# musyoku/wavenet

Measured on AMD Instinct MI355X. Metric: audio samples/sec: train fwd+bwd, 4x10-layer dilated stack (cfg2), higher is better.
Workload: dtype f32 storage+accumulate / fp16x2 split products (2^-21)

## Files before the change

wavenet_amd/csrc/mfma_gemm_b3.hip:

```cpp
#include "mfma_gemm.hpp"
#include "split_w.hpp"
#include "h2_ops.hpp"
#include <type_traits>

namespace wn {

template <bool WMAX>
__global__ void k_split_w(CGArgs a, int mode, int mtiles, int chunks_per_src, __bf16* __restrict__ img, int one) {
    if (WMAX) {
        const float mw = split_w_tile<true>(a, mode, mtiles, chunks_per_src, img, one, (int)blockIdx.x, 1.f);
        if (threadIdx.x == 0) atomicMax(const_cast<unsigned*>(a.wmax_dev), __float_as_uint(mw));
    } else {
        split_w_tile<false>(a, mode, mtiles, chunks_per_src, img, one, (int)blockIdx.x, one == 3 ? h2_scale(a.wmax_dev, kH2ScaleW) : 1.f);
    }
}

__device__ __forceinline__ int b3_ch(int r, int h) { return (r & 3) + 8 * (r >> 2) + 4 * h; }

struct RowMap { long long row[4]; bool ok[4]; };

__device__ __forceinline__ RowMap row_map(long long no, bool nvalid, int lane) {
    RowMap m;
#pragma unroll
    for (int it = 0; it < 4; ++it) {
// ... 600 lines not shown
    const long long img_stride = (long long)mtiles * kH2qTB;
    auto dma_half = [&](int s) {
        const int ss = s < nhalf ? s : nhalf - 1;
        const char* base = reinterpret_cast<const char*>(img) + (long long)(ss >> 1) * img_stride + (ss & 1) * kH2qHalf;
#pragma unroll
        for (int tt = 0; tt < 2; ++tt)
            asm_dma2(tile_off[tt], base, lds0 + ((s & 3) * MT + swave + 4 * tt) * kH2qHalf);
    };
    f32x4 xr[4][2];
    const int rs0 = rbase + a.soff[0];
    const bool rv0 = rs0 >= 0 && rs0 < a.rows_src_per_b;
    const float msk0 = rv0 ? 1.f : 0.f;
    const unsigned x_off = (unsigned)(((rb0 + (rv0 ? rs0 : 0)) * (a.ldx ? a.ldx : a.K[0]) + 8 * h) * 4);
    const char* x0 = reinterpret_cast<const char*>(a.X[0]);
    auto load_x = [&](int s, auto slot_tag) {
        constexpr int slot = decltype(slot_tag)::value;
        const int ss = s < nhalf ? s : nhalf - 1;
        const char* base = x0 + (long long)(ss >> 1) * x_stride + (ss & 1) * 64;
        asm_load16s(xr[slot][0], x_off, base);
        asm_load16s(xr[slot][1], x_off + 16, base);
    };
    f16x8 xh[2], xm[2];
    auto split_one = [&](const f32x4 (&raw)[2], float ms, int e, f16x8& oh, f16x8& om) {
        const float v = raw[e >> 2][e & 3];
        _Float16 a0, a1;
        split2h(act_apply_t<ACT>(v) * (ms * h2sx), a0, a1);
        oh[e] = a0; om[e] = a1;
    };
    using I0 = std::integral_constant<int, 0>;
    using I1 = std::integral_constant<int, 1>;
    using I2 = std::integral_constant<int, 2>;
    using I3 = std::integral_constant<int, 3>;
    load_x(0, I0{});
    asm volatile("s_waitcnt vmcnt(0)" : "+v"(xr[0][0]), "+v"(xr[0][1]) : : "memory");
#pragma unroll
    for (int e = 0; e < 8; ++e) split_one(xr[0], msk0, e, xh[0], xm[0]);
    asm volatile("" : "+v"(xh[0]), "+v"(xm[0]));
    dma_half(0); load_x(1, I1{});
    dma_half(1); load_x(2, I2{});
    dma_half(2); load_x(3, I3{});

    auto step = [&](int s, auto p_tag) {
        constexpr int p = decltype(p_tag)::value;
        constexpr int set = p & 1, nxt = 1 - set;
        constexpr int rn = (p + 1) & 3;
        asm volatile("s_waitcnt vmcnt(12)" : "+v"(xr[rn][0]), "+v"(xr[rn][1]) : : "memory");
        const float ms = msk0;
        asm volatile("s_waitcnt lgkmcnt(0)" ::: "memory");
        __builtin_amdgcn_s_barrier();
        dma_half(s + 3);
        const char* Ab = ldsq + (p * MT) * kH2qHalf + lane * 16;
        f16x8 fr[2][2];
        auto ldA = [&](int mt, f16x8 (&f)[2]) {
            f[0] = *reinterpret_cast<const f16x8*>(Ab + mt * kH2qHalf);
            f[1] = *reinterpret_cast<const f16x8*>(Ab + mt * kH2qHalf + 1024);
        };
        ldA(0, fr[0]);
#pragma unroll
        for (int mt = 0; mt < MT; ++mt) {
            f16x8 (&f)[2] = fr[mt & 1];
            asm volatile("" ::"v"(f[0]));
            asm volatile("" ::"v"(f[1]));
            if (mt + 1 < MT) ldA(mt + 1, fr[(mt + 1) & 1]);
            __builtin_amdgcn_sched_barrier(0);
            split_one(xr[rn], ms, mt, nxt ? xh[1] : xh[0], nxt ? xm[1] : xm[0]);
            acc[mt] = __builtin_amdgcn_mfma_f32_32x32x16_f16(f[1], xh[set], acc[mt], 0, 0, 0);
            acc[mt] = __builtin_amdgcn_mfma_f32_32x32x16_f16(f[0], xm[set], acc[mt], 0, 0, 0);
            acc[mt] = __builtin_amdgcn_mfma_f32_32x32x16_f16(f[0], xh[set], acc[mt], 0, 0, 0);
            __builtin_amdgcn_sched_barrier(0);
        }
        asm volatile("" : "+v"(xh[nxt]), "+v"(xm[nxt]));
        load_x(s + 4, p_tag);
    };
    for (int s = 0; s < nhalf; s += 4) {
        step(s, I0{});
        step(s + 1, I1{});
        step(s + 2, I2{});
        step(s + 3, I3{});
    }
    asm volatile("s_waitcnt vmcnt(0)"
                 : "+v"(xr[0][0]), "+v"(xr[0][1]), "+v"(xr[1][0]), "+v"(xr[1][1]), "+v"(xr[2][0]), "+v"(xr[2][1]),
                   "+v"(xr[3][0]), "+v"(xr[3][1])
                 :
                 : "memory");
#pragma unroll
    for (int mt = 0; mt < MT; ++mt)
#pragma unroll
        for (int r = 0; r < 16; ++r) acc[mt][r] *= 1.f / (h2sw * h2sx);
    __syncthreads();
    float* patch = reinterpret_cast<float*>(ldsq) + wave * 1024;
    const RowMap rm = row_map(no, nvalid, lane);
#pragma unroll
    for (int mt = 0; mt < MT; ++mt) {
        if (t0 + mt >= mtiles) break;
        float* __restrict__ og = (MODE == 2) ? a.out[t0 + mt] : a.out[0];
        const int col = (MODE == 2) ? 0 : (t0 + mt) * 32;
        float4 t[4], v[4], u[4];
#pragma unroll
        for (int q = 0; q < 4; ++q) t[q] = make_float4(acc[mt][4 * q], acc[mt][4 * q + 1], acc[mt][4 * q + 2], acc[mt][4 * q + 3]);
        if (MODE == 0 && a.gate_x) {
            rows_load(a.gate_x, a.ldo, col, rm, lane, v);
            rows_to_tile(patch, lane, v, u);
#pragma unroll
            for (int q = 0; q < 4; ++q) {
                t[q].x *= act_grad(u[q].x, a.gate_act); t[q].y *= act_grad(u[q].y, a.gate_act);
                t[q].z *= act_grad(u[q].z, a.gate_act); t[q].w *= act_grad(u[q].w, a.gate_act);
            }
        }
        if (MODE == 0 && a.residual) {
            rows_load(a.residual, a.ldo, col, rm, lane, v);
            rows_to_tile(patch, lane, v, u);
#pragma unroll
            for (int q = 0; q < 4; ++q) { t[q].x += u[q].x; t[q].y += u[q].y; t[q].z += u[q].z; t[q].w += u[q].w; }
        }
        if (a.accumulate) {
            rows_load(og, a.ldo, col, rm, lane, v);
            rows_to_tile(patch, lane, v, u);
#pragma unroll
            for (int q = 0; q < 4; ++q) { t[q].x += u[q].x; t[q].y += u[q].y; t[q].z += u[q].z; t[q].w += u[q].w; }
        }
        tile_store_rows(patch, lane, t, og, a.ldo, col, rm);
    }
}

static constexpr int kWsTile = 32 * 1024;
static constexpr int kWsLds = 2 * kWsTile + 8 * 4096;
static constexpr int kWsAhead = 2;

__global__ __launch_bounds__(512, 1) void k_dz_ws(CGArgs a, const __bf16* __restrict__ img, int mtiles, int ntiles, int nranges) {
    extern __shared__ __attribute__((aligned(16))) char ldsw[];
    const float h2sx = h2_scale(a.xmax_dev, kH2ScaleX);
    const float h2sw = h2_scale(a.wmax_dev, kH2ScaleW);
    const int tid = threadIdx.x, lane = tid & 63;
    const int wave = __builtin_amdgcn_readfirstlane(tid >> 6);
    const int j = lane & 31, h = lane >> 5;
    int range, grp;
    {
        const int ng = (mtiles + 7) >> 3;
        const int id = blockIdx.x;
        const int full = nranges & ~7;
        if (id < full * ng) {
            const int g = id / (8 * ng), rem = id - g * 8 * ng;
            range = g * 8 + (rem & 7);
            grp = rem >> 3;
        } else {
            const int t = id - full * ng;
            grp = t % ng;
            range = full + t / ng;
        }
    }
    const int t_lo = (int)((long long)range * ntiles / nranges), t_hi = (int)((long long)(range + 1) * ntiles / nranges);
    if (t_lo >= t_hi) return;
    const int layer = grp * 8 + wave;
    const bool live = layer < mtiles;
    const int N = (int)a.N, rows_out = a.rows_out_per_b, rows_src = a.rows_src_per_b, shift = a.off + a.soff[0];
    const int ldo = a.ldo;
    const long long ldx = a.ldx ? a.ldx : a.K[0];
    const float* __restrict__ X = a.X[0];
    float* __restrict__ og = a.out[live ? layer : 0];

    f16x8 A[16][2];
    {
        const char* ip = reinterpret_cast<const char*>(img) + (long long)(live ? layer : mtiles - 1) * kH2qTB + lane * 16;
#pragma unroll
        for (int kk = 0; kk < 16; ++kk)
#pragma unroll
            for (int pl = 0; pl < 2; ++pl)
                A[kk][pl] = *reinterpret_cast<const f16x8*>(ip + (long long)(kk >> 1) * mtiles * kH2qTB + (kk & 1) * kH2qHalf + pl * 1024);
    }

    auto advance = [&](int& n, int& b, int& r, int by) {
        n += by; r += by;
        const bool wrap = r >= rows_out;
        r -= wrap ? rows_out : 0;
        b += wrap ? 1 : 0;
    };
    const int lcol = (tid & 7) | ((tid >> 7) << 3), kseg = (tid >> 3) & 15;
    int ln = t_lo * 32 + lcol, lb = ln / rows_out, lr = ln - lb * rows_out;
    float4 raw[4];
    float rsc = 0.f;
    auto load_raw = [&]() {
        const int rs = lr + shift;
        const bool rv = ln < N && rs >= 0 && rs < rows_src;
        rsc = rv ? h2sx : 0.f;
        const float* p = X + (rv ? (long long)lb * rows_src + rs : 0ll) * ldx + 16 * kseg;
#pragma unroll
        for (int i = 0; i < 4; ++i) raw[i] = reinterpret_cast<const float4*>(p)[i];
        advance(ln, lb, lr, 32);
    };
    auto split_write = [&](char* buf) {
        float v[16];
#pragma unroll
        for (int e = 0; e < 16; ++e) {
            const float x = (e & 3) == 0 ? raw[e >> 2].x : (e & 3) == 1 ? raw[e >> 2].y : (e & 3) == 2 ? raw[e >> 2].z : raw[e >> 2].w;
            v[e] = fminf(fmaxf(x * rsc, -65000.f), 65000.f);
        }
        H2Op o;
        lb_split16(v, 1.f, o);
        char* d = buf + kseg * 2048 + lcol * 16;
        *reinterpret_cast<f16x8*>(d) = o.h[0];
        *reinterpret_cast<f16x8*>(d + 512) = o.h[1];
        *reinterpret_cast<f16x8*>(d + 1024) = o.m[0];
        *reinterpret_cast<f16x8*>(d + 1536) = o.m[1];
    };
    float* patch = reinterpret_cast<float*>(ldsw + 2 * kWsTile) + wave * 1024;
    const int orows = a.out_rows_per_b ? a.out_rows_per_b : rows_out, orow0 = a.out_rows_per_b ? a.out_row0 : 0;
    int sn[4], sb[4], sr[4];
#pragma unroll
    for (int it = 0; it < 4; ++it) {
        sn[it] = t_lo * 32 + it * 8 + (lane >> 3);
        sb[it] = sn[it] / rows_out;
        sr[it] = sn[it] - sb[it] * rows_out;
    }
    float4 pv0, pv1, pv2, pv3;
    auto patch_read = [&]() {
        pv0 = *reinterpret_cast<const float4*>(patch_rows(patch, lane, 0));
        pv1 = *reinterpret_cast<const float4*>(patch_rows(patch, lane, 1));
        pv2 = *reinterpret_cast<const float4*>(patch_rows(patch, lane, 2));
        pv3 = *reinterpret_cast<const float4*>(patch_rows(patch, lane, 3));
    };
    auto store_rows = [&](const float4 v, int& n, int& b, int& r, bool en) {
        const long long no = (long long)b * orows + orow0 + r;
        if (en && n < N) *reinterpret_cast<float4*>(og + no * ldo + ((lane & 7) << 2)) = v;
        advance(n, b, r, en ? 32 : 0);
    };
    auto store_tile = [&](bool en) {
        store_rows(pv0, sn[0], sb[0], sr[0], en);
        store_rows(pv1, sn[1], sb[1], sr[1], en);
        store_rows(pv2, sn[2], sb[2], sr[2], en);
        store_rows(pv3, sn[3], sb[3], sr[3], en);
    };

    f32x16 acc;
#pragma unroll
    for (int r = 0; r < 16; ++r) acc[r] = 0.f;
    const float inv = 1.f / (h2sw * h2sx);

    auto step = [&](auto live_tag, int t) {
        constexpr bool LIVE = decltype(live_tag)::value;
        char* nxt = ldsw + ((t - t_lo + 1) & 1) * kWsTile;
        const char* rd = ldsw + ((t - t_lo) & 1) * kWsTile + lane * 16;
        f16x8 fr[kWsAhead + 1][2];
        auto ldB = [&](int kk, f16x8 (&f)[2]) {
            f[0] = *reinterpret_cast<const f16x8*>(rd + kk * 2048);
            f[1] = *reinterpret_cast<const f16x8*>(rd + kk * 2048 + 1024);
        };
        if (LIVE) {
#pragma unroll
            for (int kk = 0; kk < kWsAhead; ++kk) ldB(kk, fr[kk]);
        }
#pragma unroll
        for (int kk = 0; kk < 16; ++kk) {
            if (LIVE) {
                f16x8 (&f)[2] = fr[kk % (kWsAhead + 1)];
                asm volatile("" ::"v"(f[0]));
                asm volatile("" ::"v"(f[1]));
                if (kk + kWsAhead < 16) ldB(kk + kWsAhead, fr[(kk + kWsAhead) % (kWsAhead + 1)]);
                __builtin_amdgcn_sched_barrier(0);
                acc = __builtin_amdgcn_mfma_f32_32x32x16_f16(A[kk][1], f[0], acc, 0, 0, 0);
                acc = __builtin_amdgcn_mfma_f32_32x32x16_f16(A[kk][0], f[1], acc, 0, 0, 0);
                acc = __builtin_amdgcn_mfma_f32_32x32x16_f16(A[kk][0], f[0], acc, 0, 0, 0);
                __builtin_amdgcn_sched_barrier(0);
            }
            if (kk == 5) {
                split_write(nxt);
                __builtin_amdgcn_sched_barrier(0);
            }
            if (kk == 6 && LIVE) {
                patch_read();
                __builtin_amdgcn_sched_barrier(0);
            }
            if (kk == 7) {
                if (LIVE) store_tile(t > t_lo);
                load_raw();
                __builtin_amdgcn_sched_barrier(0);
            }
        }
        if (LIVE) {
#pragma unroll
            for (int q = 0; q < 4; ++q)
                *reinterpret_cast<float4*>(patch_tile(patch, j, h, q)) =
                    make_float4(acc[4 * q] * inv, acc[4 * q + 1] * inv, acc[4 * q + 2] * inv, acc[4 * q + 3] * inv);
#pragma unroll
            for (int r = 0; r < 16; ++r) acc[r] = 0.f;
        }
        asm volatile("s_waitcnt lgkmcnt(0)" ::: "memory");
        __builtin_amdgcn_s_barrier();
    };

    load_raw();
    split_write(ldsw);
    load_raw();
    asm volatile("s_waitcnt lgkmcnt(0)" ::: "memory");
    __builtin_amdgcn_s_barrier();
    if (live) {
        for (int t = t_lo; t < t_hi; ++t) step(std::true_type{}, t);
        patch_read();
        store_tile(true);
    } else {
        for (int t = t_lo; t < t_hi; ++t) step(std::false_type{}, t);
    }
}

int launch_colgemm_b3(Call& c, CGArgs& a, int mode, int nprob, hipStream_t s) {
    if (mode != 0 && mode != 2 && mode != 3 && mode != 4 && mode != 5 && mode != 6) return WN_ESHAPE;
    if (mode == 6 && !(c.fp16x2() && a.M == 256 && a.nsrc == 1 && a.xent_target && a.xent_loss && a.out[0] &&
                       cdiv(a.N, 128) <= kXentBlocks))
        return WN_ESHAPE;
    int mtiles, nchunks, cps;
    if (mode == 0 || mode >= 3) {
        if (a.M % 32) return WN_ESHAPE;
        if ((mode == 3 || mode == 5) && a.nsrc > WN_GATE_TAPS) return WN_ESHAPE;
        if (mode == 5 && !(c.one_term() && a.M == 128 && a.ldo == 128)) return WN_ESHAPE;
        for (int i = 0; i < a.nsrc; ++i)
            if (a.K[i] != a.K[0] || a.K[i] % 32) return WN_ESHAPE;
        mtiles = ((mode == 3 || mode == 5) ? 2 : 1) * a.M / 32;
        cps = a.K[0] / 32;
        nchunks = a.nsrc * cps;
    } else {
        if (a.M != 32 || a.K[0] % 32) return WN_ESHAPE;
        mtiles = nprob;
        cps = a.K[0] / 32;
        nchunks = cps;
    }
    const bool one = c.one_term();
    const bool h2 = c.fp16x2() && ((a.h2_ok || a.xmax_dev) && (mode == 0 || mode == 2) || mode == 6);
    const size_t bytes = (size_t)nchunks * mtiles * (one ? kTileBytes / 3 : (h2 ? kTileBytes * 2 / 3 : kTileBytes));
    const size_t bytes2 = mode == 5 ? (size_t)16 * (kTileBytes / 3) : 0;
    const __bf16* pimg = nullptr; const unsigned* pwmax = nullptr;
    const bool planned = plan_split_image(c, a, mode, mtiles, cps, nchunks, one ? 1 : (h2 ? 3 : 0), bytes, &pimg, &pwmax);
    __bf16* img = planned ? const_cast<__bf16*>(pimg)
                          : reinterpret_cast<__bf16*>(c.scratch(bytes + bytes2, "the split weight image"));
    if (!img) return WN_EARG;
    if (planned) {
        a.wmax_dev = pwmax;
    } else {
    if (h2) {
        bool fresh = false;
        unsigned* wm = c.word(reinterpret_cast<const char*>(a.W[0]) + (((unsigned)mode & 7u) << 8 | ((unsigned)a.nsrc & 255u)), &fresh, s);
        if (!wm) return WN_EARG;
        a.wmax_dev = wm;
        if (fresh) hipLaunchKernelGGL(k_split_w<true>, dim3(nchunks * mtiles), dim3(256), 0, s, a, mode, mtiles, cps, img, 3);
    }
    hipLaunchKernelGGL(k_split_w<false>, dim3(nchunks * mtiles), dim3(256), 0, s, a, mode, mtiles, cps, img, one ? 1 : (h2 ? 3 : 0));
    }
    if (mode == 5) {
        if (!a.proj_W || !a.residual || !a.gate_z || a.act != WN_ACT_NONE || mtiles != 8) {
            wn::set_error("colgemm_b3: fused-layer mode needs Wp, the residual input, z and 128 gate channels");
            return WN_EARG;
        }
        CGArgs b{};
        b.nsrc = 1; b.W[0] = a.proj_W; b.wsm[0] = 128; b.wsk = 1; b.K[0] = 128; b.M = 128;
        __bf16* img2 = reinterpret_cast<__bf16*>(reinterpret_cast<char*>(img) + bytes);
        hipLaunchKernelGGL(k_split_w<false>, dim3(16), dim3(256), 0, s, b, 0, 4, 4, img2, 1);
        hipLaunchKernelGGL((k_colgemm_b3<5, WN_ACT_NONE, 1, 8>), dim3(cdiv(a.N, 128)), dim3(256), 0, s, a,
                           (const __bf16*)img, mtiles, nchunks, cps, (const __bf16*)img2);
        WN_LAUNCH_CHECK();
        return WN_OK;
    }
    if (h2 && mode == 2 && nchunks == 8 && a.ldo == 32 && !a.accumulate && !c.flag(WN_EXEC_NO_PIPELINED_GEMM) &&
        a.N < (1ll << 30) && a.rows_out_per_b >= 32 &&
        (a.N / a.rows_out_per_b + 2) * (long long)(a.out_rows_per_b > a.rows_out_per_b ? a.out_rows_per_b : a.rows_out_per_b) < (1ll << 31)) {
        int dev = 0;
        WN_HIP(hipGetDevice(&dev));
        static int capacity[64];
        if (dev < 0 || dev >= 64) { wn::set_error("colgemm_b3: device index %d", dev); return WN_ESHAPE; }
        if (!capacity[dev]) {
            int n_cu = 0, per_cu = 0;
            WN_HIP(hipDeviceGetAttribute(&n_cu, hipDeviceAttributeMultiprocessorCount, dev));
            WN_HIP(hipFuncSetAttribute(reinterpret_cast<const void*>(k_dz_ws), hipFuncAttributeMaxDynamicSharedMemorySize, kWsLds));
            WN_HIP(hipOccupancyMaxActiveBlocksPerMultiprocessor(&per_cu, k_dz_ws, 512, kWsLds));
            capacity[dev] = n_cu * per_cu > 0 ? n_cu * per_cu : -1;
        }
        const int ng = cdiv(mtiles, 8), ntiles = cdiv(a.N, 32);
        int nranges = capacity[dev] / ng;
        if (nranges > ntiles) nranges = ntiles;
        if (nranges >= 1) {
            hipLaunchKernelGGL(k_dz_ws, dim3(ng * nranges), dim3(512), kWsLds, s, a, (const __bf16*)img, mtiles, ntiles, nranges);
            WN_LAUNCH_CHECK();
            return WN_OK;
        }
    }
    const bool mt8 = (one || h2) && mtiles >= 8;
    dim3 grid(cdiv(a.N, 128) * cdiv(mtiles, mt8 ? 8 : 4));
    if (mode == 6) {
#define X_LAUNCH(ACT_, ROWS_) hipLaunchKernelGGL((k_colgemm_b3<6, ACT_, 3, 8, ROWS_>), grid, dim3(256), 0, s, a, (const __bf16*)img, \
                                                 mtiles, nchunks, cps, (const __bf16*)nullptr)
        if (c.flag(WN_EXEC_HEAD_ROW_NLL)) {
            if (a.act == WN_ACT_RELU) X_LAUNCH(WN_ACT_RELU, true);
            else if (a.act == WN_ACT_ELU) X_LAUNCH(WN_ACT_ELU, true);
            else X_LAUNCH(WN_ACT_NONE, true);
        } else if (a.act == WN_ACT_RELU) X_LAUNCH(WN_ACT_RELU, false);
        else if (a.act == WN_ACT_ELU) X_LAUNCH(WN_ACT_ELU, false);
        else X_LAUNCH(WN_ACT_NONE, false);
#undef X_LAUNCH
        WN_LAUNCH_CHECK();
        return WN_OK;
    }
#define CG_LAUNCH(MODE_, ACT_)                                                                                          \
    do {                                                                                                                \
        if (mt8) hipLaunchKernelGGL((k_colgemm_b3<MODE_, ACT_, 1, 8>), grid, dim3(256), 0, s, a, (const __bf16*)img,    \
                                    mtiles, nchunks, cps, (const __bf16*)nullptr);                                      \
        else if (one) hipLaunchKernelGGL((k_colgemm_b3<MODE_, ACT_, 1, 4>), grid, dim3(256), 0, s, a,                   \
                                         (const __bf16*)img, mtiles, nchunks, cps, (const __bf16*)nullptr);             \
        else hipLaunchKernelGGL((k_colgemm_b3<MODE_, ACT_, 6, 4>), grid, dim3(256), 0, s, a, (const __bf16*)img,        \
                                mtiles, nchunks, cps, (const __bf16*)nullptr);                                          \
    } while (0)
#define CG_LAUNCH_H2(MODE_, ACT_)                                                                                       \
    do {                                                                                                                \
        if (mt8) hipLaunchKernelGGL((k_colgemm_b3<MODE_, ACT_, 3, 8>), grid, dim3(256), 0, s, a, (const __bf16*)img,    \
                                    mtiles, nchunks, cps, (const __bf16*)nullptr);                                      \
        else hipLaunchKernelGGL((k_colgemm_b3<MODE_, ACT_, 3, 4>), grid, dim3(256), 0, s, a, (const __bf16*)img,        \
                                mtiles, nchunks, cps, (const __bf16*)nullptr);                                          \
    } while (0)
    long long x_stride = 128;
    bool lean = h2 && mt8 && mode == 0 && (nchunks & 1) == 0 && !c.flag(WN_EXEC_NO_PIPELINED_GEMM) &&
                (a.N / a.rows_out_per_b + 1) * (long long)a.rows_src_per_b * (a.ldx ? a.ldx : a.K[0]) * 4 < (1ll << 32);
    if (lean && mode == 0 && a.nsrc > 1) {
        x_stride = (const char*)a.X[1] - (const char*)a.X[0];
        lean = cps == 1;
        for (int i = 1; i < a.nsrc && lean; ++i)
            lean = a.soff[i] == a.soff[0] && a.K[i] == a.K[0] && (const char*)a.X[i] - (const char*)a.X[i - 1] == x_stride;
    } else if (lean && mode == 0) {
        lean = a.nsrc == 1;
    }
    if (lean) {
        WN_MAX_LDS_ONCE(kH2qLds, k_colgemm_h2q<0, WN_ACT_NONE>, k_colgemm_h2q<0, WN_ACT_RELU>, k_colgemm_h2q<0, WN_ACT_ELU>);
#define Q_LAUNCH(MODE_, ACT_)                                                                                 \
    hipLaunchKernelGGL((k_colgemm_h2q<MODE_, ACT_>), grid, dim3(256), kH2qLds, s, a, (const __bf16*)img, mtiles, nchunks, x_stride)
        if (a.act == WN_ACT_RELU) Q_LAUNCH(0, WN_ACT_RELU);
        else if (a.act == WN_ACT_ELU) Q_LAUNCH(0, WN_ACT_ELU);
        else Q_LAUNCH(0, WN_ACT_NONE);
#undef Q_LAUNCH
        WN_LAUNCH_CHECK();
        return WN_OK;
    }
    if (h2) {
        if (mode == 2) CG_LAUNCH_H2(2, WN_ACT_NONE);
        else if (a.act == WN_ACT_RELU) CG_LAUNCH_H2(0, WN_ACT_RELU);
        else if (a.act == WN_ACT_ELU) CG_LAUNCH_H2(0, WN_ACT_ELU);
        else CG_LAUNCH_H2(0, WN_ACT_NONE);
        WN_LAUNCH_CHECK();
        return WN_OK;
    }
#undef CG_LAUNCH_H2
    if (mode == 3) {
        if (a.act != WN_ACT_NONE || !a.gate_z) { wn::set_error("colgemm_b3: gate mode takes no activation and needs gate_z"); return WN_EARG; }
        CG_LAUNCH(3, WN_ACT_NONE);
    } else if (mode == 4) {
        if (a.act != WN_ACT_NONE || !a.gate_z || !a.gate_f || !a.gate_s) { wn::set_error("colgemm_b3: gate-backward mode needs f, s and the output"); return WN_EARG; }
        CG_LAUNCH(4, WN_ACT_NONE);
    } else if (mode == 0) {
        if (a.outmax_dev) plan_xmax_written(c, a.out[0]);
        if (a.act == WN_ACT_RELU) CG_LAUNCH(0, WN_ACT_RELU);
        else if (a.act == WN_ACT_ELU) CG_LAUNCH(0, WN_ACT_ELU);
        else if (a.act == WN_ACT_NONE) CG_LAUNCH(0, WN_ACT_NONE);
        else { wn::set_error("colgemm_b3: unknown activation %d", a.act); return WN_EARG; }
    } else {
        if (a.act != WN_ACT_NONE) { wn::set_error("colgemm_b3: multi-problem mode takes no activation"); return WN_EARG; }
        CG_LAUNCH(2, WN_ACT_NONE);
    }
#undef CG_LAUNCH
    WN_LAUNCH_CHECK();
    return WN_OK;
}

template <int MT, bool HAS_B2, int ACT, bool ONE>
__global__ __launch_bounds__(256, 2) void k_wgrad_b3(WGArgs a) {
    __shared__ __attribute__((aligned(16))) char lds[MT * kTileBytes];
    constexpr int NF = MT / 2 > 0 ? MT / 2 : 1;
    const int tid = threadIdx.x, lane = tid & 63, wv = tid >> 6;
    const int j = lane & 31, h = lane >> 5;
    const int p = blockIdx.y * 4 + wv;
    const bool active = p < a.nprob;
    const int m0 = blockIdx.z * (MT * 32);
    const int b = blockIdx.x / a.wgs_per_b;
    const int r_begin = (blockIdx.x - b * a.wgs_per_b) * a.rows_per_wg;
    const int r_end = min(a.rows_A_per_b, r_begin + a.rows_per_wg);
    const float* __restrict__ Ab = a.A + ((long long)b * a.rows_A_per_b) * a.lda + m0;
    const float* __restrict__ Bb = a.Bp[active ? p : 0] + ((long long)b * a.rows_B_per_b + a.off) * a.ldb + j;
    const float* __restrict__ B2b = a.B2p[active ? p : 0] ? a.B2p[active ? p : 0] + ((long long)b * a.rows_B_per_b + a.off) * a.ldb + j : nullptr;
    f32x16 acc[MT];
#pragma unroll
    for (int mt = 0; mt < MT; ++mt)
#pragma unroll
        for (int r = 0; r < 16; ++r) acc[mt][r] = 0.f;

    float ar[NF][8], br[2][8], b2r[2][8];
    const float* __restrict__ B2s = HAS_B2 ? B2b : Bb;
    const float amask = active ? 1.f : 0.f;
    int fm[NF], fg[NF];
#pragma unroll
    for (int it = 0; it < NF; ++it) {
        const int f = it * 256 + tid;
        fm[it] = f % (MT * 32);
        fg[it] = f / (MT * 32);
    }
    auto issue = [&](int r0) {
        const bool full = r0 + 32 <= r_end && r0 + a.off >= 0 && r0 + 31 + a.off < a.rows_B_per_b;
        if (full) {
#pragma unroll
            for (int it = 0; it < NF; ++it) {
                const float* ap = Ab + (long long)(r0 + 8 * (fg[it] & 3)) * a.lda + fm[it];
#pragma unroll
                for (int jj = 0; jj < 8; ++jj) ar[it][jj] = ap[(long long)jj * a.lda];
            }
            const float* bp = Bb + (long long)(r0 + 8 * h) * a.ldb;
            const float* b2p = B2s + (long long)(r0 + 8 * h) * a.ldb;
#pragma unroll
            for (int ks = 0; ks < 2; ++ks)
#pragma unroll
                for (int jj = 0; jj < 8; ++jj) {
                    br[ks][jj] = bp[(long long)(16 * ks + jj) * a.ldb];
                    if (HAS_B2) b2r[ks][jj] = b2p[(long long)(16 * ks + jj) * a.ldb];
                }
            return;
        }
#pragma unroll
        for (int it = 0; it < NF; ++it)
#pragma unroll
            for (int jj = 0; jj < 8; ++jj) {
                const int r = r0 + 8 * (fg[it] & 3) + jj;
                const int rc = r < r_end ? r : r_end - 1;
                ar[it][jj] = Ab[(long long)rc * a.lda + fm[it]];
            }
#pragma unroll
        for (int ks = 0; ks < 2; ++ks)
#pragma unroll
            for (int jj = 0; jj < 8; ++jj) {
                const int r = r0 + 16 * ks + 8 * h + jj;
                int rc = r < r_end ? r : r_end - 1;
                if (rc + a.off < 0) rc = -a.off;
                if (rc + a.off >= a.rows_B_per_b) rc = a.rows_B_per_b - 1 - a.off;
                br[ks][jj] = Bb[(long long)rc * a.ldb];
                if (HAS_B2) b2r[ks][jj] = B2s[(long long)rc * a.ldb];
            }
    };
    if (r_begin < r_end) issue(r_begin);
    for (int r0 = r_begin; r0 < r_end; r0 += 32) {
        bf16x8 ah[NF], am[NF], al[NF], bh[2], bm[2], bl[2];
        const bool edge = !(r0 + 32 <= r_end && r0 + a.off >= 0 && r0 + 31 + a.off < a.rows_B_per_b);
#pragma unroll
        for (int it = 0; it < NF; ++it)
#pragma unroll
            for (int e = 0; e < 8; ++e) {
                float av = ar[it][e];
                if (edge) av *= (r0 + 8 * (fg[it] & 3) + e) < r_end ? 1.f : 0.f;
                __bf16 x0, x1, x2;
                split3(av, x0, x1, x2);
                ah[it][e] = x0; am[it][e] = x1; al[it][e] = x2;
            }
#pragma unroll
        for (int ks = 0; ks < 2; ++ks)
#pragma unroll
            for (int e = 0; e < 8; ++e) {
                float bv = act_apply_t<ACT>(br[ks][e]) * amask;
                if (HAS_B2) bv *= b2r[ks][e];
                if (edge) {
                    const int rb = r0 + 16 * ks + 8 * h + e;
                    bv *= (rb < r_end && rb + a.off >= 0 && rb + a.off < a.rows_B_per_b) ? 1.f : 0.f;
                }
                __bf16 x0, x1, x2;
                split3(bv, x0, x1, x2);
                bh[ks][e] = x0; bm[ks][e] = x1; bl[ks][e] = x2;
            }
        __syncthreads();
#pragma unroll
        for (int it = 0; it < NF; ++it) {
            const int f = it * 256 + tid;
            const int m = f % (MT * 32), g = f / (MT * 32);
            if (MT >= 2 || g < 4) {
                char* d = lds + (m >> 5) * kTileBytes + ((g >> 1) * 3) * 1024 + ((m & 31) + 32 * (g & 1)) * 16;
                *reinterpret_cast<bf16x8*>(d) = ah[it];
                *reinterpret_cast<bf16x8*>(d + 1024) = am[it];
                *reinterpret_cast<bf16x8*>(d + 2048) = al[it];
            }
        }
        __syncthreads();
        if (r0 + 32 < r_end) issue(r0 + 32);
        const char* Al = lds + lane * 16;
#pragma unroll
        for (int mt = 0; mt < MT; ++mt) {
#pragma unroll
            for (int ks = 0; ks < 2; ++ks) {
                const char* q = Al + mt * kTileBytes + ks * 3 * 1024;
                const bf16x8 xh = *reinterpret_cast<const bf16x8*>(q);
                const bf16x8 xm = *reinterpret_cast<const bf16x8*>(q + 1024);
                const bf16x8 xl = *reinterpret_cast<const bf16x8*>(q + 2048);
                if (!ONE) {
                    acc[mt] = __builtin_amdgcn_mfma_f32_32x32x16_bf16(xl, bh[ks], acc[mt], 0, 0, 0);
                    acc[mt] = __builtin_amdgcn_mfma_f32_32x32x16_bf16(xh, bl[ks], acc[mt], 0, 0, 0);
                    acc[mt] = __builtin_amdgcn_mfma_f32_32x32x16_bf16(xm, bm[ks], acc[mt], 0, 0, 0);
                    acc[mt] = __builtin_amdgcn_mfma_f32_32x32x16_bf16(xm, bh[ks], acc[mt], 0, 0, 0);
                    acc[mt] = __builtin_amdgcn_mfma_f32_32x32x16_bf16(xh, bm[ks], acc[mt], 0, 0, 0);
                }
                acc[mt] = __builtin_amdgcn_mfma_f32_32x32x16_bf16(xh, bh[ks], acc[mt], 0, 0, 0);
            }
        }
    }
    if (!active) return;
    if (a.fixed_part) {
        const long long M = (long long)gridDim.z * (MT * 32);
        float* __restrict__ q = a.fixed_part + (((long long)blockIdx.x * a.nprob + p) * M) * 32 + j;
#pragma unroll
        for (int mt = 0; mt < MT; ++mt)
#pragma unroll
            for (int r = 0; r < 16; ++r) q[(long long)(m0 + mt * 32 + b3_ch(r, h)) * 32] = acc[mt][r];
        return;
    }
    float* __restrict__ o = a.out[p];
#pragma unroll
    for (int mt = 0; mt < MT; ++mt)
#pragma unroll
        for (int r = 0; r < 16; ++r)
            atomicAdd(o + (long long)(m0 + mt * 32 + b3_ch(r, h)) * a.ldo + (long long)j * (a.osk ? a.osk : 1), acc[mt][r]);
}

template <bool HAS_B2, int ACT, int TM>
__global__ __launch_bounds__(512, 1) void k_wgrad_b3w(WGArgs a) {
    constexpr int MT = 8;
    constexpr bool ONE = TM == 1;
    constexpr bool H2 = TM == 3;
    const float h2sa = H2 ? h2_scale(a.amax_dev, 1.f) : 1.f;
    const float h2sb = H2 ? h2_scale(a.bmax_dev, kH2ScaleX) : 1.f;
    extern __shared__ __attribute__((aligned(16))) char ldsw[];
    const int tid = threadIdx.x, lane = tid & 63, wv = tid >> 6;
    const int j = lane & 31, h = lane >> 5;
    const int p = blockIdx.y * 8 + wv;
    const bool active = p < a.nprob;
    const int off = a.off + a.offp[active ? p : 0];
    const int b = blockIdx.x / a.wgs_per_b;
    const int r_begin = (blockIdx.x - b * a.wgs_per_b) * a.rows_per_wg;
    const int r_end = min(a.rows_A_per_b, r_begin + a.rows_per_wg);
    const float* __restrict__ Ab = a.A + ((long long)b * a.rows_A_per_b) * a.lda;
    const float* __restrict__ Bb = a.Bp[active ? p : 0] + ((long long)b * a.rows_B_per_b + off) * a.ldb + j;
    const float* __restrict__ B2b = a.B2p[active ? p : 0] ? a.B2p[active ? p : 0] + ((long long)b * a.rows_B_per_b + off) * a.ldb + j : nullptr;
    f32x16 acc[MT];
#pragma unroll
    for (int mt = 0; mt < MT; ++mt)
#pragma unroll
        for (int r = 0; r < 16; ++r) acc[mt][r] = 0.f;

    const int fm = tid & 255;
    const int fhh = tid >> 8;
    float ar[2][8], br[2][8], b2r[2][8];
    const float* __restrict__ B2s = HAS_B2 ? B2b : Bb;
    auto issue = [&](int r0) {
        const bool full = r0 + 32 <= r_end && r0 + off >= 0 && r0 + 31 + off < a.rows_B_per_b;
        if (full) {
#pragma unroll
            for (int ks = 0; ks < 2; ++ks) {
                const float* ap = Ab + (long long)(r0 + 16 * ks + 8 * fhh) * a.lda + fm;
#pragma unroll
                for (int jj = 0; jj < 8; ++jj) ar[ks][jj] = ap[(long long)jj * a.lda];
            }
            const float* bp = Bb + (long long)(r0 + 8 * h) * a.ldb;
            const float* b2p = B2s + (long long)(r0 + 8 * h) * a.ldb;
#pragma unroll
            for (int ks = 0; ks < 2; ++ks)
#pragma unroll
                for (int jj = 0; jj < 8; ++jj) {
                    br[ks][jj] = bp[(long long)(16 * ks + jj) * a.ldb];
                    if (HAS_B2) b2r[ks][jj] = b2p[(long long)(16 * ks + jj) * a.ldb];
                }
            return;
        }
#pragma unroll
        for (int ks = 0; ks < 2; ++ks)
#pragma unroll
            for (int jj = 0; jj < 8; ++jj) {
                const int r = r0 + 16 * ks + 8 * fhh + jj;
                const int rc = r < r_end ? r : r_end - 1;
                ar[ks][jj] = Ab[(long long)rc * a.lda + fm];
            }
#pragma unroll
        for (int ks = 0; ks < 2; ++ks)
#pragma unroll
            for (int jj = 0; jj < 8; ++jj) {
                const int r = r0 + 16 * ks + 8 * h + jj;
                int rc = r < r_end ? r : r_end - 1;
                if (rc + off < 0) rc = -off;
// ... 388 lines not shown
```

Measured before the change: 48.37 million.

## Add persistent weight-stationary pipelined kernel for 256x256 three-term dX GEMM

Result: faster. 48.88 million, median of 6 (+1.0%).

```diff
diff --git a/wavenet_amd/csrc/mfma_gemm_b3.hip b/wavenet_amd/csrc/mfma_gemm_b3.hip
--- a/wavenet_amd/csrc/mfma_gemm_b3.hip
+++ b/wavenet_amd/csrc/mfma_gemm_b3.hip
@@ -926,6 +926,186 @@
     }
 }
 
+static constexpr int kDxTile = 48 * 1024;
+static constexpr int kDxLds = 2 * kDxTile + 4 * 4096;
+static constexpr int kDxAhead = 2;
+
+template <int ACT>
+__global__ __launch_bounds__(256, 1) void k_dx_ws(CGArgs a, const __bf16* __restrict__ img, int ntiles, int nranges) {
+    extern __shared__ __attribute__((aligned(16))) char ldsx[];
+    const int tid = threadIdx.x, lane = tid & 63;
+    const int wave = __builtin_amdgcn_readfirstlane(tid >> 6);
+    const int j = lane & 31, h = lane >> 5;
+    int range, grp;
+    {
+        const int id = blockIdx.x;
+        const int full = nranges & ~7;
+        if (id < full * 2) {
+            const int g = id >> 4, rem = id & 15;
+            range = g * 8 + (rem & 7);
+            grp = rem >> 3;
+        } else {
+            const int t = id - full * 2;
+            grp = t & 1;
+            range = full + (t >> 1);
+        }
+    }
+    const int t_lo = (int)((long long)range * ntiles / nranges), t_hi = (int)((long long)(range + 1) * ntiles / nranges);
+    if (t_lo >= t_hi) return;
+    const int mtile = grp * 4 + wave;
+    const int N = (int)a.N;
+    const float* __restrict__ X = a.X[0];
+    const float* __restrict__ G = a.gate_x;
+    float* __restrict__ og = a.out[0] + mtile * 32 + ((lane & 7) << 2);
+    unsigned* const outmax = a.outmax_dev;
+
+    bf16x8 A[16][3];
+    {
+        const char* ip = reinterpret_cast<const char*>(img) + (long long)mtile * kTileBytes + lane * 16;
+#pragma unroll
+        for (int kk = 0; kk < 16; ++kk)
+#pragma unroll
+            for (int pl = 0; pl < 3; ++pl)
+                A[kk][pl] = *reinterpret_cast<const bf16x8*>(ip + (long long)(kk >> 1) * 8 * kTileBytes + (kk & 1) * (kTileBytes / 2) + pl * 1024);
+    }
+
+    const int lcol = (tid & 7) | ((tid >> 7) << 3), kseg = (tid >> 3) & 15;
+    int ln = t_lo * 32 + lcol;
+    float4 raw[2][4];
+    bool rok[2] = {false, false};
+    auto load_raw = [&]() {
+#pragma unroll
+        for (int c2 = 0; c2 < 2; ++c2) {
+            const int n = ln + 16 * c2;
+            rok[c2] = n < N;
+            const float* p = X + (long long)(rok[c2] ? n : 0) * 256 + 16 * kseg;
+#pragma unroll
+            for (int i = 0; i < 4; ++i) raw[c2][i] = reinterpret_cast<const float4*>(p)[i];
+        }
+        ln += 32;
+    };
+    auto split_write = [&](char* buf, int q) {
+        const int c2 = q >> 1, half = q & 1;
+        bf16x8 ph, pm, pl;
+#pragma unroll
+        for (int e = 0; e < 8; ++e) {
+            const float4 r = raw[c2][2 * half + (e >> 2)];
+            const float x = (e & 3) == 0 ? r.x : (e & 3) == 1 ? r.y : (e & 3) == 2 ? r.z : r.w;
+            __bf16 hh, mm, ll;
+            split3(rok[c2] ? x : 0.f, hh, mm, ll);
+            ph[e] = hh; pm[e] = mm; pl[e] = ll;
+        }
+        char* d = buf + kseg * 3072 + (lcol + 16 * c2 + 32 * half) * 16;
+        *reinterpret_cast<bf16x8*>(d) = ph;
+        *reinterpret_cast<bf16x8*>(d + 1024) = pm;
+        *reinterpret_cast<bf16x8*>(d + 2048) = pl;
+    };
+    float* patch = reinterpret_cast<float*>(ldsx + 2 * kDxTile) + wave * 1024;
+    float4 pv[4], gv[4];
+    float omax = 0.f;
+    auto patch_read = [&]() {
+#pragma unroll
+        for (int it = 0; it < 4; ++it) pv[it] = *reinterpret_cast<const float4*>(patch_rows(patch, lane, it));
+    };
+    auto load_gate = [&](int t) {
+        if (ACT == WN_ACT_NONE) return;
+#pragma unroll
+        for (int it = 0; it < 4; ++it) {
+            const int n = t * 32 + it * 8 + (lane >> 3);
+            gv[it] = *reinterpret_cast<const float4*>(G + (long long)(n < N ? n : 0) * 256 + mtile * 32 + ((lane & 7) << 2));
+        }
+    };
+    auto store_tile = [&](int t) {
+#pragma unroll
+        for (int it = 0; it < 4; ++it) {
+            const int n = t * 32 + it * 8 + (lane >> 3);
+            float4 v = pv[it];
+            if (ACT != WN_ACT_NONE) {
+                v.x *= act_grad(gv[it].x, ACT); v.y *= act_grad(gv[it].y, ACT);
+                v.z *= act_grad(gv[it].z, ACT); v.w *= act_grad(gv[it].w, ACT);
+            }
+            if (n < N) {
+                if (outmax) omax = fmaxf(omax, fmaxf(fmaxf(fabsf(v.x), fabsf(v.y)), fmaxf(fabsf(v.z), fabsf(v.w))));
+                *reinterpret_cast<float4*>(og + (long long)n * 256) = v;
+            }
+        }
+    };
+
+    f32x16 acc;
+#pragma unroll
+    for (int r = 0; r < 16; ++r) acc[r] = 0.f;
+
+    auto step = [&](int t) {
+        char* nxt = ldsx + ((t - t_lo + 1) & 1) * kDxTile;
+        const char* rd = ldsx + ((t - t_lo) & 1) * kDxTile + lane * 16;
+        bf16x8 fr[kDxAhead + 1][3];
+        auto ldB = [&](int kk, bf16x8 (&f)[3]) {
+            f[0] = *reinterpret_cast<const bf16x8*>(rd + kk * 3072);
+            f[1] = *reinterpret_cast<const bf16x8*>(rd + kk * 3072 + 1024);
+            f[2] = *reinterpret_cast<const bf16x8*>(rd + kk * 3072 + 2048);
+        };
+#pragma unroll
+        for (int kk = 0; kk < kDxAhead; ++kk) ldB(kk, fr[kk]);
+#pragma unroll
+        for (int kk = 0; kk < 16; ++kk) {
+            bf16x8 (&f)[3] = fr[kk % (kDxAhead + 1)];
+            asm volatile("" ::"v"(f[0]));
+            asm volatile("" ::"v"(f[1]));
+            asm volatile("" ::"v"(f[2]));
+            if (kk + kDxAhead < 16) ldB(kk + kDxAhead, fr[(kk + kDxAhead) % (kDxAhead + 1)]);
+            __builtin_amdgcn_sched_barrier(0);
+            acc = __builtin_amdgcn_mfma_f32_32x32x16_bf16(A[kk][2], f[0], acc, 0, 0, 0);
+            acc = __builtin_amdgcn_mfma_f32_32x32x16_bf16(A[kk][0], f[2], acc, 0, 0, 0);
+            acc = __builtin_amdgcn_mfma_f32_32x32x16_bf16(A[kk][1], f[1], acc, 0, 0, 0);
+            acc = __builtin_amdgcn_mfma_f32_32x32x16_bf16(A[kk][1], f[0], acc, 0, 0, 0);
+            acc = __builtin_amdgcn_mfma_f32_32x32x16_bf16(A[kk][0], f[1], acc, 0, 0, 0);
+            acc = __builtin_amdgcn_mfma_f32_32x32x16_bf16(A[kk][0], f[0], acc, 0, 0, 0);
+            __builtin_amdgcn_sched_barrier(0);
+            if (kk < 4) {
+                split_write(nxt, kk);
+                __builtin_amdgcn_sched_barrier(0);
+            }
+            if (kk == 4) {
+                load_raw();
+                __builtin_amdgcn_sched_barrier(0);
+            }
+            if (kk == 6) {
+                patch_read();
+                __builtin_amdgcn_sched_barrier(0);
+            }
+            if (kk == 7) {
+                if (t > t_lo) store_tile(t - 1);
+                load_gate(t);
+                __builtin_amdgcn_sched_barrier(0);
+            }
+        }
+#pragma unroll
+        for (int q = 0; q < 4; ++q)
+            *reinterpret_cast<float4*>(patch_tile(patch, j, h, q)) = make_float4(acc[4 * q], acc[4 * q + 1], acc[4 * q + 2], acc[4 * q + 3]);
+#pragma unroll
+        for (int r = 0; r < 16; ++r) acc[r] = 0.f;
+        asm volatile("s_waitcnt lgkmcnt(0)" ::: "memory");
+        __builtin_amdgcn_s_barrier();
+    };
+
+    load_raw();
+#pragma unroll
+    for (int q = 0; q < 4; ++q) split_write(ldsx, q);
+    load_raw();
+    asm volatile("s_waitcnt lgkmcnt(0)" ::: "memory");
+    __builtin_amdgcn_s_barrier();
+    for (int t = t_lo; t < t_hi; ++t) step(t);
+    patch_read();
+    store_tile(t_hi - 1);
+    if (outmax) {
+        for (int o = 32; o >= 1; o >>= 1) omax = fmaxf(omax, __shfl_xor(omax, o));
+        if (lane == 0) {
+            const unsigned bits = __float_as_uint(omax);
+            if (bits > __hip_atomic_load(outmax, __ATOMIC_RELAXED, __HIP_MEMORY_SCOPE_AGENT)) atomicMax(outmax, bits);
+        }
+    }
+}
+
 int launch_colgemm_b3(Call& c, CGArgs& a, int mode, int nprob, hipStream_t s) {
     if (mode != 0 && mode != 2 && mode != 3 && mode != 4 && mode != 5 && mode != 6) return WN_ESHAPE;
     if (mode == 6 && !(c.fp16x2() && a.M == 256 && a.nsrc == 1 && a.xent_target && a.xent_loss && a.out[0] &&
@@ -1001,6 +1181,39 @@
         if (nranges > ntiles) nranges = ntiles;
         if (nranges >= 1) {
             hipLaunchKernelGGL(k_dz_ws, dim3(ng * nranges), dim3(512), kWsLds, s, a, (const __bf16*)img, mtiles, ntiles, nranges);
+            WN_LAUNCH_CHECK();
+            return WN_OK;
+        }
+    }
+    if (!one && !h2 && mode == 0 && a.nsrc == 1 && mtiles == 8 && nchunks == 8 && a.ldo == 256 && (a.ldx == 0 || a.ldx == 256) &&
+        !a.bias[0] && !a.residual && !a.accumulate && a.act == WN_ACT_NONE && a.off == 0 && a.soff[0] == 0 && !a.out_rows_per_b &&
+        a.N < (1ll << 30) && a.rows_out_per_b == a.N && a.rows_src_per_b == a.N && !c.flag(WN_EXEC_NO_PIPELINED_GEMM) &&
+        (!a.gate_x || a.gate_act == WN_ACT_RELU || a.gate_act == WN_ACT_ELU)) {
+        int dev = 0;
+        WN_HIP(hipGetDevice(&dev));
+        static int capacity[64];
+        if (dev < 0 || dev >= 64) { wn::set_error("colgemm_b3: device index %d", dev); return WN_ESHAPE; }
+        if (!capacity[dev]) {
+            int n_cu = 0, per_cu = 0;
+            WN_HIP(hipDeviceGetAttribute(&n_cu, hipDeviceAttributeMultiprocessorCount, dev));
+            WN_HIP(hipFuncSetAttribute(reinterpret_cast<const void*>(k_dx_ws<WN_ACT_NONE>), hipFuncAttributeMaxDynamicSharedMemorySize, kDxLds));
+            WN_HIP(hipFuncSetAttribute(reinterpret_cast<const void*>(k_dx_ws<WN_ACT_RELU>), hipFuncAttributeMaxDynamicSharedMemorySize, kDxLds));
+            WN_HIP(hipFuncSetAttribute(reinterpret_cast<const void*>(k_dx_ws<WN_ACT_ELU>), hipFuncAttributeMaxDynamicSharedMemorySize, kDxLds));
+            WN_HIP(hipOccupancyMaxActiveBlocksPerMultiprocessor(&per_cu, k_dx_ws<WN_ACT_RELU>, 256, kDxLds));
+            capacity[dev] = n_cu * per_cu > 0 ? n_cu * per_cu : -1;
+        }
+        const int ntiles = cdiv(a.N, 32);
+        int nranges = capacity[dev] / 2;
+        if (nranges > ntiles) nranges = ntiles;
+        if (nranges >= 1) {
+            if (a.outmax_dev) plan_xmax_written(c, a.out[0]);
+            const int gact = a.gate_x ? a.gate_act : WN_ACT_NONE;
+            if (gact == WN_ACT_RELU)
+                hipLaunchKernelGGL((k_dx_ws<WN_ACT_RELU>), dim3(2 * nranges), dim3(256), kDxLds, s, a, (const __bf16*)img, ntiles, nranges);
+            else if (gact == WN_ACT_ELU)
+                hipLaunchKernelGGL((k_dx_ws<WN_ACT_ELU>), dim3(2 * nranges), dim3(256), kDxLds, s, a, (const __bf16*)img, ntiles, nranges);
+            else
+                hipLaunchKernelGGL((k_dx_ws<WN_ACT_NONE>), dim3(2 * nranges), dim3(256), kDxLds, s, a, (const __bf16*)img, ntiles, nranges);
             WN_LAUNCH_CHECK();
             return WN_OK;
         }
```
